# dazchi/gym-uav-collision-avoidance

Hardware: AMD Instinct MI355X
Metric: env-steps/s (higher is better)
Workload: dtype f32+f64

## Files before the change

gym_uav_collision_avoidance_amd/csrc/uavx_device.hpp:

```cpp
#pragma once
#include <hip/hip_runtime.h>
#include <stdint.h>

namespace uavx {

constexpr int kWave = 64;
#ifndef UAVX_BLOCK
#define UAVX_BLOCK 64
#endif
constexpr int kBlock = UAVX_BLOCK;
constexpr int kWavesPerBlock = kBlock / kWave;
constexpr float kPi = 3.14159265358979323846f;
constexpr float kInvPi = 0.318309886183790671538f;
constexpr float kTwoPi = 6.28318530717958647692f;
constexpr float kInvTwoPi = 0.159154943091895335769f;

__device__ __forceinline__ void wave_lds_sync() {
    __builtin_amdgcn_fence(__ATOMIC_RELEASE, "wavefront");
    __builtin_amdgcn_wave_barrier();
    __builtin_amdgcn_fence(__ATOMIC_ACQUIRE, "wavefront");
}

using rsrc_t = __amdgpu_buffer_rsrc_t;
typedef unsigned int u32x4 __attribute__((ext_vector_type(4)));
typedef unsigned int u32x2 __attribute__((ext_vector_type(2)));
constexpr int kAuxSc1 = 16;

__device__ __forceinline__ rsrc_t make_rsrc(const void *base, uint32_t bytes) {
    return __builtin_amdgcn_make_buffer_rsrc(const_cast<void *>(base),  0, (int)bytes, 0x00020000);
}
__device__ __forceinline__ void store16_wt(rsrc_t r, uint32_t byte_off, float4 v) {
    u32x4 d = {__float_as_uint(v.x), __float_as_uint(v.y), __float_as_uint(v.z), __float_as_uint(v.w)};
    __builtin_amdgcn_raw_buffer_store_b128(d, r, (int)byte_off, 0, kAuxSc1);
}
__device__ __forceinline__ void store16_wt(rsrc_t r, uint32_t byte_off, double2 v) {
    const unsigned long long a = __double_as_longlong(v.x), b = __double_as_longlong(v.y);
    u32x4 d = {(unsigned)a, (unsigned)(a >> 32), (unsigned)b, (unsigned)(b >> 32)};
    __builtin_amdgcn_raw_buffer_store_b128(d, r, (int)byte_off, 0, kAuxSc1);
}
__device__ __forceinline__ void store8_wt(rsrc_t r, uint32_t byte_off, float2 v) {
    u32x2 d = {__float_as_uint(v.x), __float_as_uint(v.y)};
    __builtin_amdgcn_raw_buffer_store_b64(d, r, (int)byte_off, 0, kAuxSc1);
}

typedef const __attribute__((address_space(4))) char *karg_ptr;
__device__ __forceinline__ karg_ptr late_kargs() {
    karg_ptr ka = (karg_ptr)__builtin_amdgcn_kernarg_segment_ptr();
    asm volatile("" : "+s"(ka));
    return ka;
}
template <class T>
__device__ __forceinline__ T late_karg(uint32_t byte_off, karg_ptr ka = late_kargs()) {
    return *(const __attribute__((address_space(4))) T *)(ka + byte_off);
}

__device__ __forceinline__ float sqrt_rn(float s) {
    if (__builtin_expect(__any((__float_as_uint(s) - 1u) < 0x0F7FFFFFu), 0)) return sqrtf(s);
    const float r = __builtin_amdgcn_sqrtf(s);
    const float lo = __uint_as_float(__float_as_uint(r) - 1u), hi = __uint_as_float(__float_as_uint(r) + 1u);
    const float e_lo = fmaf(-lo, r, s), e_hi = fmaf(-hi, r, s);
    float out = (e_lo <= 0.f) ? lo : r;
    out = (e_hi > 0.f) ? hi : out;
    return out;
}

__device__ __forceinline__ float norm32(float x, float y) {
    float a = x * x;
    float b = y * y;
    return sqrt_rn(a + b);
}

__device__ __forceinline__ double clip64(double x, double lo, double hi) {
    double m = (x < lo) ? lo : x;
    return (m > hi) ? hi : m;
}

__device__ __forceinline__ float wrap_pi(float x) {
    float k = rintf(x * kInvTwoPi);
    return fmaf(-k, kTwoPi, x);
}

__device__ __forceinline__ float atan2_fast(float y, float x) {
    const float ax = fabsf(x), ay = fabsf(y);
    const float mx = fmaxf(ax, ay), mn = fminf(ax, ay);
    const bool big = mn > 0.41421356237f * mx;
    const float num = big ? mn - mx : mn;
    float den = big ? mn + mx : mx;
    den = (mx == 0.f) ? 1.f : den;
    const float t = num * __builtin_amdgcn_rcpf(den);
    const float z = t * t;
    float pl = fmaf(8.05374449538e-2f, z, -1.38776856032e-1f);
    pl = fmaf(pl, z, 1.99777106478e-1f);
    pl = fmaf(pl, z, -3.33329491539e-1f);
    float r = fmaf(pl * z, t, t);
    r = big ? r + 0.78539816339744830962f : r;
    r = (ay > ax) ? 1.57079632679489661923f - r : r;
    r = (x < 0.f) ? kPi - r : r;
    return copysignf(r, y);
}

__device__ __forceinline__ float atan2_exact(float y, float x) {
    const float ax = fabsf(x), ay = fabsf(y);
    const float mx = fmaxf(ax, ay), mn = fminf(ax, ay);
    const bool big = mn > 0.41421356237f * mx;
    const float num = big ? mn - mx : mn;
    float den = big ? mn + mx : mx;
    den = (mx == 0.f) ? 1.f : den;
    const float t = num / den;
    const float z = t * t;
    float pl = fmaf(8.05374449538e-2f, z, -1.38776856032e-1f);
    pl = fmaf(pl, z, 1.99777106478e-1f);
    pl = fmaf(pl, z, -3.33329491539e-1f);
    float r = fmaf(pl * z, t, t);
    r = big ? r + 0.78539816339744830962f : r;
    r = (ay > ax) ? 1.57079632679489661923f - r : r;
    r = (x < 0.f) ? kPi - r : r;
    return copysignf(r, y);
}

__device__ __forceinline__ double max64u(double x, double lim) {
    double r;
    asm("v_max_f64 %0, %1, %2" : "=v"(r) : "v"(x), "s"(lim));
    return r;
}
__device__ __forceinline__ double min64u(double x, double lim) {
    double r;
    asm("v_min_f64 %0, %1, %2" : "=v"(r) : "v"(x), "s"(lim));
    return r;
}

__device__ __forceinline__ double div_tau(double x, double tau, double rtau, bool recip_ok) {
    if (!recip_ok) return x / tau;
    x = min64u(max64u(x, -1e300), 1e300);
    const double q0 = x * rtau;
    const double rem = fma(-q0, tau, x);
    return fma(rem, rtau, q0);
}

__device__ __forceinline__ void axis_update(double a, double tau, double rtau, bool recip_ok, double amax, double vmax,
                                            double &v, float &x) {
    const bool poisoned = __builtin_isunordered(a, v);
    const double dv = min64u(max64u(div_tau(a - v, tau, rtau, recip_ok), -amax), amax);
    double nv = min64u(max64u(v + dv * tau, -vmax), vmax);
    nv = poisoned ? __builtin_nan("") : nv;
    v = nv;
    x = (float)((double)x + v * tau);
}

__device__ __forceinline__ void sincospi32(float t, float &sn, float &cs) {
    const float k = rintf(2.0f * t);
    const float r = fmaf(-0.5f, k, t);
    const float z = r * r;
    float ps = fmaf(z, 0.0821458866f, -0.599264529f);
    ps = fmaf(ps, z, 2.55016404f);
    ps = fmaf(ps, z, -5.16771278f);
    ps = fmaf(ps, z, 3.14159265f);
    ps = ps * r;
    float pc = fmaf(z, -0.0258068913f, 0.235330630f);
    pc = fmaf(pc, z, -1.33526277f);
    pc = fmaf(pc, z, 4.05871213f);
    pc = fmaf(pc, z, -4.93480220f);
    pc = fmaf(pc, z, 1.0f);
    const int q = (int)k & 3;
    sn = (q == 0) ? ps : (q == 1) ? pc : (q == 2) ? -ps : -pc;
    cs = (q == 0) ? pc : (q == 1) ? -ps : (q == 2) ? -pc : ps;
}

__device__ __forceinline__ void sincos_ref(double x, double &sn, double &cs) {
    const double ax = fabs(x);
    if (__builtin_expect(__any(ax > 823549.6561538912), 0)) {
        if (ax > 823549.6561538912) { sincos(x, &sn, &cs); return; }
    }
    const double fn = rint(x * 6.36619772367581382433e-01);
    const int n = (int)fn;
    double r = x - fn * 1.57079632673412561417e+00;
    double t = r;
    double w = fn * 6.07710050630396597660e-11;
    r = t - w;
    w = fn * 2.02226624879595063154e-21 - ((t - r) - w);
    t = r;
    w = fn * 2.02226624871116645580e-21;
    r = t - w;
    w = fn * 8.47842766036889956997e-32 - ((t - r) - w);
    const double y0 = r - w;
    const double y1 = (r - y0) - w;
    const double z = y0 * y0, zz = z * z, v = z * y0;
    const double rs = 8.33333333332248946124e-03 + z * (-1.98412698298579493134e-04 + z * 2.75573137070700676789e-06) +
                      z * zz * (-2.50507602534068634195e-08 + z * 1.58969099521155010221e-10);
    const double ks = y0 - ((z * (0.5 * y1 - v * rs) - y1) - v * -1.66666666666666324348e-01);
    const double rc = z * (4.16666666666666019037e-02 + z * (-1.38888888888741095749e-03 + z * 2.48015872894767294178e-05)) +
                      zz * zz * (-2.75573143513906633035e-07 + z * (2.08757232129817482790e-09 + z * -1.13596475577881948265e-11));
    const double hz = 0.5 * z, wc = 1.0 - hz;
    const double kc = wc + (((1.0 - wc) - hz) + (z * rc - y0 * y1));
    const int q = n & 3;
    double s_ = (q == 0) ? ks : (q == 1) ? kc : (q == 2) ? -ks : -kc;
    double c_ = (q == 0) ? kc : (q == 1) ? -ks : (q == 2) ? -kc : ks;
    const bool tiny = ax < 7.450580596923828125e-9;
    s_ = tiny ? x : s_;
    c_ = tiny ? 1.0 : c_;
    const bool fin = ax <= 1.7976931348623157e308;
    sn = fin ? s_ : __builtin_nan("");
    cs = fin ? c_ : __builtin_nan("");
}

__device__ __forceinline__ void polar_to_command_ref32(float a0, float a1, float h, double &ax, double &ay) {
    const float u = a0 * 0.5f + 0.5f;
    const float v = u * h;
    const float theta = a1 * 3.14159265358979323846f;
    double s, c;
    sincos_ref((double)theta, s, c);
    ax = (double)(v * (float)c);
    ay = (double)(v * (float)s);
}
__device__ __forceinline__ void polar_to_command_ref64(double a0, double a1, float h, double &ax, double &ay) {
    const double v = (a0 * 0.5 + 0.5) * (double)h;
    const double theta = a1 * 3.14159265358979323846;
    double s, c;
    sincos_ref(theta, s, c);
    ax = v * c;
    ay = v * s;
}
template <bool ACT64>
__device__ __forceinline__ void polar_to_command_ref(float h, double &ax, double &ay) {
    if (ACT64) polar_to_command_ref64(ax, ay, h, ax, ay);
    else polar_to_command_ref32((float)ax, (float)ay, h, ax, ay);
}

__device__ __forceinline__ void philox4x32(uint32_t c0, uint32_t c1, uint32_t c2, uint32_t c3, uint32_t k0,
                                           uint32_t k1, uint32_t out[4]) {
#pragma unroll
    for (int r = 0; r < 10; r++) {
        uint64_t p0 = (uint64_t)0xD2511F53u * c0;
        uint64_t p1 = (uint64_t)0xCD9E8D57u * c2;
        uint32_t n0 = (uint32_t)(p1 >> 32) ^ c1 ^ k0;
        uint32_t n1 = (uint32_t)p1;
        uint32_t n2 = (uint32_t)(p0 >> 32) ^ c3 ^ k1;
        uint32_t n3 = (uint32_t)p0;
        c0 = n0; c1 = n1; c2 = n2; c3 = n3;
        k0 += 0x9E3779B9u; k1 += 0xBB67AE85u;
    }
    out[0] = c0; out[1] = c1; out[2] = c2; out[3] = c3;
}
__device__ __forceinline__ double bits53(uint32_t a, uint32_t b) {
    return ((double)(a >> 5) * 67108864.0 + (double)(b >> 6)) / 9007199254740992.0;
}
struct ResetCandidates {
    float sx, sy, tx, ty;
};
// ... 41 lines not shown
```

gym_uav_collision_avoidance_amd/csrc/uavx_multi.hip:

```cpp
#include <hip/hip_runtime.h>

#include <cmath>
#include <cstddef>
#include <cstdio>
#include <cstdlib>
#include <cstring>
#include <new>
#include <string>
#include <type_traits>

#include "../../include/uavx.h"
#include "uavx_device.hpp"

namespace uavx {

#ifndef UAVX_LATE
#define UAVX_LATE 1
#endif
template <bool ON>
__device__ __forceinline__ karg_ptr kargs_if() {
    if constexpr (ON && UAVX_LATE) return late_kargs();
    else return nullptr;
}
template <bool ON, class T>
// ... 147 lines not shown
    m.cnt = (int)envs_here * N;
    return m;
}
template <int NT, bool EXT = false, int W = 1>
__device__ __forceinline__ LaneMap lane_map(const MultiParams &p, uint32_t wave = blockIdx.x) {
    return lane_map_from<NT, EXT, W>((uint32_t)p.E, p.N, p.epw, p.magic, p.nslots, wave);
}

struct AgentRegs {
    float x, y, prev_d;
    uint32_t flags;
    float tx, ty, init_d;
    double vx, vy;
};

template <bool EXT, int W = 1>
struct LdsT {
    static constexpr int kW = W;
    static constexpr int kRows = (EXT && kExtSlots > kWave * W) ? kExtSlots : kWave * W;
    float4 pos[kRows];
    float theta[kRows];
    float obs[kWave * W * UAVX_OBS_DIM];
};
template <>
struct LdsT<true, 1> {
    static constexpr int kW = 1;
    static constexpr int kRows = kExtSlots;
    union {
        struct {
            float4 pos[kRows];
            float theta[kRows];
        };
        float obs[kWave * UAVX_OBS_DIM];
    };
};
template <int W>
__device__ __forceinline__ void group_sync() {
    if (W == 1) wave_lds_sync();
    else __syncthreads();
}
template <int W>
__device__ __forceinline__ bool group_any(bool v) {
    if (W == 1) return __ballot(v) != 0ull;
    return __syncthreads_or(v ? 1 : 0) != 0;
}
using Lds = LdsT<false>;
template <int T>
struct LdsTiles {
    static constexpr int kW = 1;
    static constexpr int kRows = kWave * T;
    float4 pos[kRows];
    float theta[kRows];
    float obs[kWave * T * UAVX_OBS_DIM];
};

template <bool EXT>
__device__ __forceinline__ float sense_limit(const MultiParams &p, uint32_t flags) {
    if (EXT && p.n_levels > 0) return p.levels[(flags & kLevelMask) >> kLevelShift].sq_sense;
    return p.sq_sense;
}
template <bool EXT>
__device__ __forceinline__ WorldLims world_lims(const MultiParams &p, uint32_t flags) {
    WorldLims w;
    if (EXT && p.n_levels > 0) {
        const float4 *t = reinterpret_cast<const float4 *>(&p.levels[(flags & kLevelMask) >> kLevelShift]);
        const float4 a = t[0], b = t[1];
        w.lo_x = a.x; w.lo_y = a.y; w.hi_x = a.z; w.hi_y = a.w;
        w.sq_sense = b.x; w.sq_two_r = b.y; w.inv_sense = b.z; w.inv_diag = b.w;
    } else {
        w.lo_x = p.lo_x; w.lo_y = p.lo_y; w.hi_x = p.hi_x; w.hi_y = p.hi_y;
        w.sq_sense = p.sq_sense; w.sq_two_r = p.sq_two_r; w.inv_sense = p.inv_sense; w.inv_diag = p.inv_diag;
    }
    return w;
}

__device__ __forceinline__ float natural_prev_d(uint32_t flags, float x, float y, float tx, float ty) {
    const float d = norm32(tx - x, ty - y);
    return ((flags & UAVX_FLAG_DONE) && !(flags & kFlagJustDone)) ? 0.f : d;
}

__device__ __forceinline__ void load_agent(const MultiParams &p, uint32_t a, AgentRegs &s) {
    const float2 d = p.pos[a];
    const double2 v = p.vel[a];
    const Goal g = p.goal[a];
    s.x = d.x; s.y = d.y;
    s.vx = v.x; s.vy = v.y;
    s.tx = g.tx; s.ty = g.ty; s.init_d = g.init_d; s.flags = g.flags;
    s.prev_d = natural_prev_d(s.flags, s.x, s.y, s.tx, s.ty);
    if (s.flags & kFlagPrevOvr) s.prev_d = p.prev_ovr[a];
}
__device__ __forceinline__ void store_agent(const MultiParams &p, float2 *pos, double2 *vel, Goal *goal, uint32_t a,
                                            const AgentRegs &s, uint32_t flags_in) {
    store16_wt(make_rsrc(vel, (uint32_t)p.E * (uint32_t)p.N * 16u), a * 16u, make_double2(s.vx, s.vy));
    pos[a] = make_float2(s.x, s.y);
    if (s.flags != flags_in) goal[a].flags = s.flags;
}
__device__ __forceinline__ void store_agent(const MultiParams &p, uint32_t a, const AgentRegs &s, uint32_t flags_in) {
    store_agent(p, p.pos, p.vel, p.goal, a, s, flags_in);
}

struct Neigh {
    float d1, d2;
    int j1, j2;
    float step_sq_min;
};

template <int NT, bool STEP, class LDS>
__device__ __forceinline__ Neigh scan_neighbours_exact(float sq_sense, const LaneMap &m, const LDS &lds, float nx,
                                                       float ny) {
    const int N = NT ? NT : m.nslots;
    Neigh r;
    r.d1 = r.d2 = INFINITY;
    r.j1 = r.j2 = -1;
    r.step_sq_min = INFINITY;
    const float4 *row = &lds.pos[m.rbase];
    auto visit = [&](int j, float4 q) {
        const float dxn = q.z - nx, dyn = q.w - ny;
        const float ax = dxn * dxn, ay = dyn * dyn;
        const float sn = ax + ay;
        if (STEP) {
            const float dxo = q.x - nx, dyo = q.y - ny;
            const float bx = dxo * dxo, by = dyo * dyo;
            const float so = bx + by;
            const float ss = (j < m.i) ? sn : so;
            r.step_sq_min = fminf(r.step_sq_min, (ss < sq_sense) ? ss : INFINITY);
        }
        const float dn = (sn < sq_sense) ? sqrt_rn(sn) : INFINITY;
        const bool lt1 = dn < r.d1, lt2 = dn < r.d2;
        r.d2 = lt1 ? r.d1 : (lt2 ? dn : r.d2);
        r.j2 = lt1 ? r.j1 : (lt2 ? j : r.j2);
        r.d1 = lt1 ? dn : r.d1;
        r.j1 = lt1 ? j : r.j1;
    };
    if (NT) {
        constexpr int M = NT > 1 ? NT - 1 : 1;
        float4 q[M];
        int js[M];
#pragma unroll
        for (int k = 0; k < NT - 1; k++) {
            js[k] = k + (k >= m.i ? 1 : 0);
            q[k] = row[js[k]];
        }
#pragma unroll
        for (int k = 0; k < NT - 1; k++) visit(js[k], q[k]);
    } else {
        for (int k = 0; k < N - 1; k++) {
            const int j = k + (k >= m.i ? 1 : 0);
            visit(j, row[j]);
        }
    }
    return r;
}

#ifdef UAVX_STAMPS
__shared__ int g_dbg_fallback;
#endif
__device__ __forceinline__ uint32_t med3_u32(uint32_t a, uint32_t b, uint32_t c) {
    uint32_t r;
    asm("v_med3_u32 %0, %1, %2, %3" : "=v"(r) : "v"(a), "v"(b), "v"(c));
    return r;
}

template <int NT, bool STEP, class LDS>
__device__ __forceinline__ Neigh scan_neighbours(float sq_sense, const LaneMap &m, const LDS &lds, float nx,
                                                 float ny) {
    if (NT != 0 && NT <= 5) return scan_neighbours_exact<NT, STEP>(sq_sense, m, lds, nx, ny);
    const int N = NT ? NT : m.nslots;
    if (NT == 0 && N <= 5) return scan_neighbours_exact<NT, STEP>(sq_sense, m, lds, nx, ny);
    const float4 *row = &lds.pos[m.rbase];
    uint32_t k1 = 0xffffffffu, k2 = 0xffffffffu, k3 = 0xffffffffu;
    float step_min = INFINITY;
    uint32_t keep;
    asm("v_mov_b32 %0, 0xffffffc0" : "=v"(keep));
    auto visit = [&](uint32_t c, bool below, float4 q) {
        const float dxn = q.z - nx, dyn = q.w - ny;
        const float ax = dxn * dxn, ay = dyn * dyn;
        const float sn = ax + ay;
        if (STEP) {
            const float dxo = q.x - nx, dyo = q.y - ny;
            const float bx = dxo * dxo, by = dyo * dyo;
            const float so = bx + by;
            step_min = fminf(step_min, below ? sn : so);
        }
        uint32_t key;
        asm("v_and_or_b32 %0, %1, %2, %3" : "=v"(key) : "v"(sn), "v"(keep), "s"(c));
        k3 = med3_u32(k2, k3, key);
        k2 = med3_u32(k1, k2, key);
        k1 = min(k1, key);
    };
    const char *rowb = reinterpret_cast<const char *>(row);
    auto other = [&](int c, bool below) {
        return *reinterpret_cast<const float4 *>(rowb + c * 16 + (below ? 0 : 16));
    };
    if (NT) {
#ifndef UAVX_SCANBATCH
#define UAVX_SCANBATCH 7
#endif
        constexpr int M = NT > 1 ? NT - 1 : 1;
        constexpr int BATCH = M < UAVX_SCANBATCH ? M : UAVX_SCANBATCH;
#pragma unroll
        for (int c0 = 0; c0 < NT - 1; c0 += BATCH) {
            float4 q[BATCH];
#pragma unroll
            for (int c = 0; c < BATCH; c++)
                if (c0 + c < NT - 1) q[c] = other(c0 + c, c0 + c < m.i);
#pragma unroll
            for (int c = 0; c < BATCH; c++)
                if (c0 + c < NT - 1) visit((uint32_t)(c0 + c), c0 + c < m.i, q[c]);
        }
    } else {
        const int NL = m.nlearn;
        int c = 0;
        for (; c + 1 < NL - 1; c += 2) {
            const bool la = c < m.i, lb = c + 1 < m.i;
            const float4 qa = other(c, la), qb = other(c + 1, lb);
            visit((uint32_t)c, la, qa);
            visit((uint32_t)c + 1u, lb, qb);
        }
        if (c < NL - 1) {
            const bool la = c < m.i;
            visit((uint32_t)c, la, other(c, la));
            c++;
        }
        auto body = [&](uint32_t c, int r) {
            const float2 q = *reinterpret_cast<const float2 *>(&row[r].z);
            const float dxn = q.x - nx, dyn = q.y - ny;
            const float ax = dxn * dxn, ay = dyn * dyn;
            const float sn = ax + ay;
            if (STEP) step_min = fminf(step_min, sn);
            uint32_t key;
            asm("v_and_or_b32 %0, %1, %2, %3" : "=v"(key) : "v"(sn), "v"(keep), "s"(c));
            k3 = med3_u32(k2, k3, key);
            k2 = med3_u32(k1, k2, key);
            k1 = min(k1, key);
        };
        for (; c + 1 < N - 1; c += 2) {
            body((uint32_t)c, c + 1);
            body((uint32_t)c + 1u, c + 2);
        }
        if (c < N - 1) body((uint32_t)c, c + 1);
    }
    const uint32_t t1 = k1 >> 6, t2 = k2 >> 6, t3 = k3 >> 6, ts = __float_as_uint(sq_sense) >> 6;
    const bool near_tie = m.active && ((t2 - t1 <= 1u && t1 <= ts) || (t3 - t2 <= 1u && t2 <= ts));
#ifdef UAVX_STAMPS
    if (__any(near_tie)) g_dbg_fallback = 1;
#endif
    const int c1 = (int)(k1 & 63u), c2 = (int)(k2 & 63u);
    const int j1 = c1 + (c1 >= m.i ? 1 : 0), j2 = c2 + (c2 >= m.i ? 1 : 0);
    const float4 q1 = row[j1], q2 = row[j2];
    const float ex1 = q1.z - nx, ey1 = q1.w - ny, ex2 = q2.z - nx, ey2 = q2.w - ny;
    const float mx1 = ex1 * ex1, my1 = ey1 * ey1, mx2 = ex2 * ex2, my2 = ey2 * ey2;
    const float s1 = mx1 + my1, s2 = mx2 + my2;
    const bool in1 = s1 < sq_sense, in2 = s2 < sq_sense;
    Neigh r;
    r.step_sq_min = (step_min < sq_sense) ? step_min : INFINITY;
    r.d1 = in1 ? sqrt_rn(s1) : INFINITY;
    r.d2 = in2 ? sqrt_rn(s2) : INFINITY;
    r.j1 = in1 ? j1 : -1;
    r.j2 = in2 ? j2 : -1;
    unsigned long long tied = __ballot(near_tie);
    if (__popcll(tied) > 6) return scan_neighbours_exact<NT, STEP>(sq_sense, m, lds, nx, ny);
    while (tied != 0ull) {
        const int tl = (int)__builtin_ctzll(tied);
        tied &= tied - 1ull;
        const float ax = __int_as_float(__builtin_amdgcn_readlane(__float_as_int(nx), tl));
        const float ay = __int_as_float(__builtin_amdgcn_readlane(__float_as_int(ny), tl));
        const float lim = __int_as_float(__builtin_amdgcn_readlane(__float_as_int(sq_sense), tl));
        const int ti = __builtin_amdgcn_readlane(m.i, tl), trb = __builtin_amdgcn_readlane(m.rbase, tl);
        const int t = (int)(threadIdx.x & (kWave - 1));
        const bool mine = t < N - 1;
        const int j = mine ? t + (t >= ti ? 1 : 0) : ti;
        const float4 q = lds.pos[trb + j];
        const float dx = q.z - ax, dy = q.w - ay;
        const float xx = dx * dx, yy = dy * dy;
        const float sn = xx + yy;
        const float dn = sqrt_rn(sn);
        unsigned long long key = (mine && sn < lim) ? ((unsigned long long)__float_as_uint(dn) << 32) | (uint32_t)j : ~0ull;
        auto wave_min = [](unsigned long long k) {
#pragma unroll
            for (int off = 32; off > 0; off >>= 1) {
                const uint32_t hi = __shfl_xor((uint32_t)(k >> 32), off), lo = __shfl_xor((uint32_t)k, off);
                const unsigned long long o = ((unsigned long long)hi << 32) | lo;
                k = o < k ? o : k;
            }
            return k;
        };
        const unsigned long long m1 = wave_min(key);
        const unsigned long long m2 = wave_min(key == m1 ? ~0ull : key);
        if (t == tl) {
            r.d1 = m1 == ~0ull ? INFINITY : __uint_as_float((uint32_t)(m1 >> 32));
            r.j1 = m1 == ~0ull ? -1 : (int)(uint32_t)m1;
            r.d2 = m2 == ~0ull ? INFINITY : __uint_as_float((uint32_t)(m2 >> 32));
            r.j2 = m2 == ~0ull ? -1 : (int)(uint32_t)m2;
        }
    }
    return r;
}

template <class LDS>
__device__ __forceinline__ void assemble_obs(const MultiParams &p, const WorldLims &w, const LaneMap &m, const LDS &lds,
                                             const Neigh &nb, float nx, float ny, float speed, float theta, float dist_t,
                                             float dth, float o[10]) {
    o[0] = speed * p.inv_vmax_norm;
    o[1] = theta * kInvPi;
    o[2] = dist_t * w.inv_diag;
    o[3] = dth * kInvPi;
    const bool has1 = nb.j1 >= 0, has2 = nb.j2 >= 0;
    const int i1 = m.rbase + (has1 ? nb.j1 : 0), i2 = m.rbase + (has2 ? nb.j2 : 0);
    const float4 q1 = lds.pos[i1], q2 = lds.pos[i2];
    const float t1 = lds.theta[i1], t2 = lds.theta[i2];
    const float b1 = wrap_pi(atan2_fast(q1.w - ny, q1.z - nx) - theta) * kInvPi;
    const float b2 = wrap_pi(atan2_fast(q2.w - ny, q2.z - nx) - theta) * kInvPi;
    const float h1 = wrap_pi(t1 - theta) * kInvPi;
    const float h2 = wrap_pi(t2 - theta) * kInvPi;
    o[4] = has1 ? nb.d1 * w.inv_sense : 1.f;
    o[5] = has1 ? b1 : 1.f;
    o[6] = has1 ? h1 : 0.f;
    o[7] = has2 ? nb.d2 * w.inv_sense : 1.f;
    o[8] = has2 ? b2 : 1.f;
    o[9] = has2 ? h2 : 0.f;
}

template <int NT, class LDS>
__device__ __forceinline__ void store_obs_block(const MultiParams &p, const LaneMap &m, LDS &lds, const float o[10],
                                                float *obs_out) {
    constexpr int T = kWave * LDS::kW;
    float *stage = lds.obs + m.obs0;
    if (m.active) {
        float2 *dst = reinterpret_cast<float2 *>(stage + m.lane * UAVX_OBS_DIM);
#pragma unroll
        for (int k = 0; k < 5; k++) dst[k] = make_float2(o[2 * k], o[2 * k + 1]);
    }
    group_sync<LDS::kW>();
    const int nfloat = m.cnt * UAVX_OBS_DIM;
    const rsrc_t r = make_rsrc(obs_out, (uint32_t)p.E * (uint32_t)p.N * (UAVX_OBS_DIM * 4u));
    const uint32_t gbase = m.a0 * (UAVX_OBS_DIM * 4u);
    if (NT ? (NT % 2 == 0) : ((p.N & 1) == 0)) {
#pragma unroll
        for (int k = 0; k < 3; k++) {
            const int f = (k * T + m.lane) * 4;
            if (f < nfloat) store16_wt(r, gbase + f * 4u, *reinterpret_cast<const float4 *>(stage + f));
        }
    } else {
        const int head = (gbase & 8u) ? 2 : 0;
        const int mid = (nfloat - head) / 4;
        const int tail = head + mid * 4;
#pragma unroll
        for (int k = 0; k < 3; k++) {
            const int q = k * T + m.lane;
            if (q < mid) {
                const float *src = stage + head + q * 4;
                const float2 lo = *reinterpret_cast<const float2 *>(src), hi = *reinterpret_cast<const float2 *>(src + 2);
                store16_wt(r, gbase + (uint32_t)(head + q * 4) * 4u, make_float4(lo.x, lo.y, hi.x, hi.y));
            }
        }
        if (m.lane == 0 && head) store8_wt(r, gbase, *reinterpret_cast<const float2 *>(stage));
        if (m.lane == 1 && tail < nfloat) store8_wt(r, gbase + (uint32_t)tail * 4u, *reinterpret_cast<const float2 *>(stage + tail));
    }
    group_sync<LDS::kW>();
}

__device__ __forceinline__ float4 make_leg(float body_step, float x, float y, float wx, float wy) {
    const float dx = wx - x, dy = wy - y;
    const float d = norm32(dx, dy);
    float4 leg = make_float4(0.f, 0.f, 0.f, 0.f);
    if (d > 0.f) {
        const float sc = body_step / d;
        leg.x = dx * sc; leg.y = dy * sc;
        leg.w = floorf(d / body_step);
    }
    leg.z = atan2_exact(dy, dx);
    return leg;
}

template <bool MOVE, class LDS, bool LATEW = false>
__device__ __forceinline__ void stage_bodies(const MultiParams &p, const LaneMap &m, LDS &lds, uint32_t flags, bool ready,
                                             uint32_t steps, uint32_t ep_draw) {
    const int L = p.N;
    const bool leveled = p.n_levels > 0;
    const LevelParams *lv = &p.levels[(flags & kLevelMask) >> kLevelShift];
    const int b_active = m.active ? (leveled ? lv->b_active : p.B) : 0;
    const uint32_t kk = steps & (uint32_t)p.body_pmask;
    const bool retarget = MOVE && steps != 0u && kk == 0u;
    const float kf = (float)kk;
#pragma unroll 1
    for (int k = 0; k < p.kb; k++) {
        const int b = k * L + m.i;
        const bool valid = m.active && b < p.B && !ready;
        const bool on = valid && b < b_active;
        const uint32_t gi = m.e * (uint32_t)p.B + (uint32_t)b;
        float2 q = make_float2(INFINITY, INFINITY);
        float4 leg = make_float4(0.f, 0.f, 0.f, 0.f);
        if (on) { q = p.body_pos[gi]; leg = p.body_leg[gi]; }
        if (on && retarget) {
            const ResetCandidates c = reset_candidates((uint64_t)LATE(LATEW, p, env_offset) + m.e, (uint32_t)(L + b),
                                                       0x80000000u | (steps >> p.body_pshift), ep_draw, LATE(LATEW, p, body_k0),
                                                       LATE(LATEW, p, body_k1), leveled ? lv->lox : LATE(LATEW, p, lox),
                                                       leveled ? lv->loy : LATE(LATEW, p, loy), leveled ? lv->hix : LATE(LATEW, p, hix),
                                                       leveled ? lv->hiy : LATE(LATEW, p, hiy));
            leg = make_leg(p.body_step, q.x, q.y, c.sx, c.sy);
            p.body_leg[gi] = leg;
        }
        if (MOVE && on && kf < leg.w) {
            q.x = q.x + leg.x; q.y = q.y + leg.y;
            p.body_pos[gi] = q;
        }
        if (valid) {
            lds.pos[m.rbase + L + b] = make_float4(q.x, q.y, q.x, q.y);
            lds.theta[m.rbase + L + b] = leg.z;
        }
    }
}

template <int NT, bool EXT, class LDS, bool LATEW = false>
__device__ __forceinline__ void step_agent(const MultiParams &p, const LaneMap &m, LDS &lds, AgentRegs &s, double ax,
                                           double ay, int evaluate, float o[10], float &rew, uint32_t &done_out,
                                           uint32_t &reach_ev, uint32_t &coll_ev, bool frozen = false,
                                           uint32_t env_steps = 0, uint32_t ep_draw = 0) {
    const float sq_sense = sense_limit<EXT>(p, s.flags);
    const bool was_done = (s.flags & UAVX_FLAG_DONE) != 0;
    const bool parked = EXT && (s.flags & kFlagInactive) != 0;
    if (!frozen) s.flags &= ~(kFlagPrevOvr | kFlagJustDone);
    const float ox = s.x, oy = s.y;
    float pd = 0.f, d = 0.f;
    if (!was_done && !frozen && !parked) {
        axis_update(ax, p.tau, p.rtau, p.recip_ok != 0, p.amax, p.vmax, s.vx, s.x);
        axis_update(ay, p.tau, p.rtau, p.recip_ok != 0, p.amax, p.vmax, s.vy, s.y);
        pd = s.prev_d;
    }
    const float tdx = s.tx - s.x, tdy = s.ty - s.y;
    const float dist_t = norm32(tdx, tdy);
    if (!was_done) d = dist_t;
    const float theta = atan2_fast((float)s.vy, (float)s.vx);
    const float dth = wrap_pi(atan2_fast(tdy, tdx) - theta);

    if (m.active) {
        lds.pos[m.rbase + m.i] = make_float4(ox, oy, s.x, s.y);
        lds.theta[m.rbase + m.i] = theta;
    }
    if (EXT && p.B > 0) stage_bodies<true, LDS, LATEW>(p, m, lds, s.flags, frozen, env_steps, ep_draw);
    group_sync<LDS::kW>();
    const Neigh nb = scan_neighbours<NT, true>(sq_sense, m, lds, s.x, s.y);
    const WorldLims w = world_lims<EXT>(p, s.flags);

    const float inv_init = __builtin_amdgcn_rcpf(s.init_d);
    float r = -0.01f * fminf(p.vmax_norm * inv_init, 1.0f);
    r += (50.0f * p.inv_vmax_norm) * (pd - d);
    const float frac = d * inv_init * (1.0f / 1.5f);
    r *= (r > 0.f) ? (1.0f - frac) : (1.0f + frac);
    r -= 0.01f * fabsf(dth);

    const bool collision = nb.step_sq_min <= w.sq_two_r;
    if (collision) r = -2.0f;
    coll_ev = 0;
    if (nb.step_sq_min <= p.sq_hard && !(s.flags & (UAVX_FLAG_DONE | UAVX_FLAG_COLLIDED)) && !frozen) {
        coll_ev = 1;
        s.flags |= UAVX_FLAG_COLLIDED;
    }
    const double sq = fma(s.vy, s.vy, s.vx * s.vx);
    const bool oob = !(s.x >= w.lo_x && s.x <= w.hi_x && s.y >= w.lo_y && s.y <= w.hi_y);
    float speed = __builtin_amdgcn_sqrtf((float)sq);
    reach_ev = 0;
    if (frozen) {
        done_out = 0;
        r = 0.f;
    } else if (d < 0.5f && !collision && sq < p.speed_sq_lim) {
        done_out = 1;
        reach_ev = was_done ? 0u : 1u;
        s.flags |= UAVX_FLAG_DONE | (was_done ? 0u : kFlagJustDone);
        const double nv = sqrt(sq);
        double fx = s.vx / nv * 0.001, fy = s.vy / nv * 0.001;
        if (fx != fx || fy != fy) { fx = 0.0; fy = 0.0; }
        s.vx = fx; s.vy = fy;
        speed = __builtin_amdgcn_sqrtf((float)fma(fy, fy, fx * fx));
        r += 10.0f;
    } else if (oob) {
        done_out = evaluate ? 0u : 1u;
    } else {
        done_out = 0;
    }
    if (!frozen) s.prev_d = d;
    rew = r;
    assemble_obs(p, w, m, lds, nb, s.x, s.y, speed, theta, dist_t, dth, o);
    if (parked) {
#pragma unroll
        for (int k = 0; k < UAVX_OBS_DIM; k++) o[k] = 0.f;
        rew = 0.f;
        done_out = frozen ? 0u : 1u;
    }
}

template <bool ACT64>
__device__ __forceinline__ void load_action(const void *__restrict__ actions, uint32_t a, double &ax, double &ay) {
    if (ACT64) {
        const double2 v = reinterpret_cast<const double2 *>(actions)[a];
        ax = v.x; ay = v.y;
    } else {
        const float2 v = reinterpret_cast<const float2 *>(actions)[a];
        ax = (double)v.x; ay = (double)v.y;
    }
}

#ifndef UAVX_STEPB
#define UAVX_STEPB 8
#endif
template <int NT, bool ACT64, bool EXT, int W, int T = 1>
__global__ __launch_bounds__(kWave * W * T, (EXT && W == 1) ? UAVX_STEPB : 1) void step_kernel(
    const void *__restrict__ actions, char *slab, uint32_t off_vel, uint32_t off_goal, uint32_t off_rec, uint32_t off_wsteps,
    uint32_t num_envs, uint32_t n_agents, uint32_t envs_per_group, uint32_t magic, uint32_t nslots, MultiParams p, int evaluate,
    float *__restrict__ obs_out, float *__restrict__ rew_out, uint8_t *__restrict__ done_out) {
    static_assert(T == 1 || W == 1, "tiles are one-wavefront workgroups side by side");
    using LDS = std::conditional_t<(T > 1), LdsTiles<T>, LdsT<EXT, W>>;
    static_assert(T == 1 || !EXT, "tiles: the plain variants only");
    __shared__ LDS lds;
    const uint32_t tile = T > 1 ? (uint32_t)__builtin_amdgcn_readfirstlane((int)(threadIdx.x / kWave)) : 0u;
    float2 *const pos_b = reinterpret_cast<float2 *>(slab);
    double2 *const vel_b = reinterpret_cast<double2 *>(slab + off_vel);
    Goal *const goal_b = reinterpret_cast<Goal *>(slab + off_goal);
    const uint32_t wave_id = blockIdx.x * T + tile;
    const LaneMap m = lane_map_from<NT, EXT, W>(num_envs, (int)n_agents, (int)envs_per_group, (int)magic, (int)nslots, wave_id,
                                                T > 1 ? threadIdx.x % kWave : threadIdx.x, tile);
    AgentRegs s = {};
    double ax = 0.0, ay = 0.0;
    uint4 rec = make_uint4(0, 0, 0, 0);
    uint32_t wave_count = 0;
    {
        const uint32_t el = m.active ? m.e : 0u, al = m.active ? m.a : 0u;
        if (EXT) {
            rec = reinterpret_cast<const uint4 *>(slab + off_rec)[el];
            wave_count = reinterpret_cast<const uint32_t *>(slab + off_wsteps)[wave_id];
        }
        load_action<ACT64>(actions, al, ax, ay);
        const float2 d = pos_b[al];
        const double2 v = vel_b[al];
        const Goal g = goal_b[al];
        __builtin_amdgcn_sched_barrier(0);
        s.x = d.x; s.y = d.y; s.vx = v.x; s.vy = v.y;
        s.tx = g.tx; s.ty = g.ty; s.init_d = g.init_d; s.flags = g.flags;
        s.prev_d = natural_prev_d(s.flags, s.x, s.y, s.tx, s.ty);
        if (m.active && (s.flags & kFlagPrevOvr)) s.prev_d = p.prev_ovr[m.a];
    }
    const uint32_t flags_in = s.flags;
    float o[10], rew;
    uint32_t dn, re, ce;
    step_agent<NT, EXT, LDS, false>(p, m, lds, s, ax, ay, evaluate, o, rew, dn, re, ce, false, wave_count - rec.x,
                                    ((rec.y & ~kRecEnded) - 1u) & ~kRecEnded);
    if (m.active) {
        if (!(EXT && (flags_in & kFlagInactive))) store_agent(p, pos_b, vel_b, goal_b, m.a, s, flags_in);
        rew_out[m.a] = rew;
        done_out[m.a] = (uint8_t)dn;
        if (re) atomicAdd(&p.reach[m.e], 1u);
        if (ce) atomicAdd(&p.coll[m.e], 1u);
        if (!(fabsf(rew) < INFINITY)) atomicAdd(&p.nonfin[m.e], 1u);
        if (m.lane == 0) {
            uint32_t *const ws = reinterpret_cast<uint32_t *>(slab + off_wsteps);
            if (EXT) ws[m.wave] = wave_count + 1u;
            else atomicAdd(&ws[m.wave], 1u);
        }
    }
    store_obs_block<NT>(p, m, lds, o, obs_out);
}

template <class LDS, class MAP>
__device__ __forceinline__ bool lowest_clash(const MAP &m, LDS &lds, unsigned long long group, bool clash, int &low) {
    if (LDS::kW == 1) {
        const unsigned long long bits = __ballot(clash);
        const unsigned long long mine = (bits >> m.base) & group;
        low = mine ? (int)__builtin_ctzll(mine) : 64;
        return bits != 0ull;
    } else {
        int *slot = reinterpret_cast<int *>(lds.obs) + m.g;
        if (m.i == 0) *slot = 64;
        __syncthreads();
        if (clash) atomicMin(slot, m.i);
        const bool any = __syncthreads_or(clash ? 1 : 0) != 0;
        low = *slot;
        return any;
    }
}

__device__ __forceinline__ bool too_close(float sq_two_r, float ax, float ay, float bx, float by) {
    const float dx = ax - bx, dy = ay - by;
    const float xx = dx * dx, yy = dy * dy;
    return xx + yy <= sq_two_r;
}

#ifndef UAVX_CHAINROWS
#define UAVX_CHAINROWS 4
#endif
constexpr int kChainRows = UAVX_CHAINROWS;
template <int NT, bool EXT, class LDS>
__device__ __forceinline__ void reset_envs_wave(const MultiParams &p, const LaneMap &m, LDS &lds, bool go,
                                                uint32_t episode, uint32_t k0, uint32_t k1, AgentRegs &s,
                                                float2 *bpos_out, float4 *bleg_out, uint8_t *lvl_out) {
    const int N = NT ? NT : p.N;
    float4 *row = &lds.pos[m.rbase];
    const uint64_t ge = (uint64_t)p.env_offset + m.e;
    const unsigned long long group = (N >= 64) ? ~0ull : ((1ull << N) - 1ull);
    double lox = p.lox, loy = p.loy, hix = p.hix, hiy = p.hiy;
    float sq2r = p.sq_two_r;
    uint32_t lvl = 0;
    int nl = N, nb = 0;
    if (EXT) {
        if (go && p.n_levels > 0) {
            if (p.level_lo >= 0) {
                uint32_t o[4];
                reset_words(ge, 0xFFFFu, 0u, episode, k0, k1, o);
                lvl = (uint32_t)p.level_lo + __umulhi(o[0], (uint32_t)(p.level_hi - p.level_lo + 1));
            } else {
                lvl = p.lvl_next[m.e];
            }
            lvl = min(lvl, (uint32_t)(p.n_levels - 1));
        }
        nb = p.B;
        if (p.n_levels > 0) {
            const LevelParams *lv = &p.levels[lvl];
            lox = lv->lox; loy = lv->loy; hix = lv->hix; hiy = lv->hiy;
            sq2r = lv->sq_two_r;
            nl = lv->n_active; nb = lv->b_active;
        }
    }
    const bool gl = go && m.i < nl;
    ResetCandidates c = {0.f, 0.f, 0.f, 0.f};
    if (gl) {
        c = reset_candidates(ge, m.i, 0u, episode, k0, k1, lox, loy, hix, hiy);
        row[m.i] = make_float4(c.sx, c.sy, c.tx, c.ty);
    }
    group_sync<LDS::kW>();
#pragma unroll 1
    for (int phase = 0; phase < 2; phase++) {
        uint32_t attempt = 0;
#pragma unroll 1
        for (;;) {
            bool clash = false;
            if (gl) {
                const float qx = phase ? c.tx : c.sx, qy = phase ? c.ty : c.sy;
                clash = phase ? too_close(sq2r, qx, qy, c.sx, c.sy) : false;
#pragma unroll 1
                for (int j0 = 0; j0 < m.i; j0 += kChainRows) {
                    float2 o[kChainRows];
#pragma unroll
                    for (int u = 0; u < kChainRows; u++) {
                        const float4 *r4 = &row[min(j0 + u, m.i - 1)];
                        o[u] = *reinterpret_cast<const float2 *>(phase ? &r4->z : &r4->x);
                    }
#pragma unroll
                    for (int u = 0; u < kChainRows; u++) clash = clash || too_close(sq2r, o[u].x, o[u].y, qx, qy);
                }
            }
            int low;
            if (!lowest_clash<LDS>(m, lds, group, clash, low)) break;
            const bool redraw = gl && m.i == low;
            group_sync<LDS::kW>();
            if (redraw) {
                const ResetCandidates r = reset_candidates(ge, m.i, ++attempt, episode, k0, k1, lox, loy, hix, hiy);
                if (phase) { c.tx = r.tx; c.ty = r.ty; row[m.i].z = c.tx; row[m.i].w = c.ty; }
                else { c.sx = r.sx; c.sy = r.sy; row[m.i].x = c.sx; row[m.i].y = c.sy; }
            }
            group_sync<LDS::kW>();
        }
    }
    if (EXT) {
#pragma unroll 1
        for (int k = 0; k < p.kb; k++) {
            const int b = k * N + m.i;
            const bool on = go && b < nb;
            const int slot = N + b;
            uint32_t attempt = 0;
            float qx = 0.f, qy = 0.f;
            if (on) {
                const ResetCandidates r = reset_candidates(ge, (uint32_t)slot, 0u, episode, k0, k1, lox, loy, hix, hiy);
                qx = r.sx; qy = r.sy;
                row[slot].x = qx; row[slot].y = qy;
            }
            group_sync<LDS::kW>();
#pragma unroll 1
            for (;;) {
                bool clash = false;
                if (on) {
                    const int cnt = nl + b;
#pragma unroll 1
                    for (int j0 = 0; j0 < cnt; j0 += kChainRows) {
                        float2 o[kChainRows];
#pragma unroll
                        for (int u = 0; u < kChainRows; u++) {
                            const int j = min(j0 + u, cnt - 1);
                            o[u] = *reinterpret_cast<const float2 *>(&row[j < nl ? j : N + (j - nl)].x);
                        }
#pragma unroll
                        for (int u = 0; u < kChainRows; u++) clash = clash || too_close(sq2r, o[u].x, o[u].y, qx, qy);
                    }
                }
                int low;
                if (!lowest_clash<LDS>(m, lds, group, clash, low)) break;
                const bool redraw = on && m.i == low;
                group_sync<LDS::kW>();
                if (redraw) {
                    const ResetCandidates r = reset_candidates(ge, (uint32_t)slot, ++attempt, episode, k0, k1, lox, loy, hix, hiy);
                    qx = r.sx; qy = r.sy;
                    row[slot].x = qx; row[slot].y = qy;
                }
                group_sync<LDS::kW>();
            }
// ... 1562 lines not shown
```

Baseline: 10.82 billion.

## Add squared-distance neighbour scan, buffer loads, cheaper atan2 and angle wrap

```diff
diff --git a/gym_uav_collision_avoidance_amd/csrc/uavx_device.hpp b/gym_uav_collision_avoidance_amd/csrc/uavx_device.hpp
--- a/gym_uav_collision_avoidance_amd/csrc/uavx_device.hpp
+++ b/gym_uav_collision_avoidance_amd/csrc/uavx_device.hpp
@@ -80,20 +80,21 @@
     return fmaf(-k, kTwoPi, x);
 }
 
+__device__ __forceinline__ float wrap_unit(float x) {
+    return fmaf(__builtin_amdgcn_fractf(fmaf(x, kInvTwoPi, 0.5f)), 2.0f, -1.0f);
+}
+
 __device__ __forceinline__ float atan2_fast(float y, float x) {
     const float ax = fabsf(x), ay = fabsf(y);
     const float mx = fmaxf(ax, ay), mn = fminf(ax, ay);
-    const bool big = mn > 0.41421356237f * mx;
-    const float num = big ? mn - mx : mn;
-    float den = big ? mn + mx : mx;
-    den = (mx == 0.f) ? 1.f : den;
-    const float t = num * __builtin_amdgcn_rcpf(den);
+    const float t = mn * __builtin_amdgcn_rcpf(fmaxf(mx, 1.17549435e-38f));
     const float z = t * t;
-    float pl = fmaf(8.05374449538e-2f, z, -1.38776856032e-1f);
-    pl = fmaf(pl, z, 1.99777106478e-1f);
-    pl = fmaf(pl, z, -3.33329491539e-1f);
+    float pl = fmaf(7.37447338e-3f, z, -3.55211943e-2f);
+    pl = fmaf(pl, z, 8.21691155e-2f);
+    pl = fmaf(pl, z, -1.33988619e-1f);
+    pl = fmaf(pl, z, 1.98618680e-1f);
+    pl = fmaf(pl, z, -3.33253950e-1f);
     float r = fmaf(pl * z, t, t);
-    r = big ? r + 0.78539816339744830962f : r;
     r = (ay > ax) ? 1.57079632679489661923f - r : r;
     r = (x < 0.f) ? kPi - r : r;
     return copysignf(r, y);
diff --git a/gym_uav_collision_avoidance_amd/csrc/uavx_multi.hip b/gym_uav_collision_avoidance_amd/csrc/uavx_multi.hip
--- a/gym_uav_collision_avoidance_amd/csrc/uavx_multi.hip
+++ b/gym_uav_collision_avoidance_amd/csrc/uavx_multi.hip
@@ -323,9 +323,6 @@
     return r;
 }
 
-#ifdef UAVX_STAMPS
-__shared__ int g_dbg_fallback;
-#endif
 __device__ __forceinline__ uint32_t med3_u32(uint32_t a, uint32_t b, uint32_t c) {
     uint32_t r;
     asm("v_med3_u32 %0, %1, %2, %3" : "=v"(r) : "v"(a), "v"(b), "v"(c));
@@ -333,8 +330,61 @@
 }
 
 template <int NT, bool STEP, class LDS>
+__device__ __forceinline__ Neigh scan_neighbours_sq(float sq_sense, const LaneMap &m, const LDS &lds, float nx, float ny) {
+    static_assert(NT == 4, "three other agents");
+    const float4 *row = &lds.pos[m.rbase];
+    constexpr uint32_t kInfBits = 0x7f800000u;
+    uint32_t s1 = kInfBits, s2 = kInfBits, s3 = kInfBits;
+    float step_min = INFINITY;
+    int j1 = -1, j2 = -1;
+    constexpr int M = NT - 1;
+    float4 q[M];
+    int js[M];
+#pragma unroll
+    for (int k = 0; k < M; k++) {
+        js[k] = k + (k >= m.i ? 1 : 0);
+        q[k] = row[js[k]];
+    }
+#pragma unroll
+    for (int k = 0; k < M; k++) {
+        const int j = js[k];
+        const float dxn = q[k].z - nx, dyn = q[k].w - ny;
+        const float ax = dxn * dxn, ay = dyn * dyn;
+        const float sn0 = ax + ay;
+        if (STEP) {
+            const float dxo = q[k].x - nx, dyo = q[k].y - ny;
+            const float bx = dxo * dxo, by = dyo * dyo;
+            const float so = bx + by;
+            step_min = fminf(step_min, (j < m.i) ? sn0 : so);
+        }
+        const uint32_t sn = (sn0 < sq_sense) ? __float_as_uint(sn0) : kInfBits;
+        const bool lt1 = sn < s1, lt2 = sn < s2;
+        j2 = lt1 ? j1 : (lt2 ? j : j2);
+        j1 = lt1 ? j : j1;
+        s3 = med3_u32(s2, s3, sn);
+        s2 = med3_u32(s1, s2, sn);
+        s1 = min(s1, sn);
+    }
+    Neigh r;
+    r.step_sq_min = (step_min < sq_sense) ? step_min : INFINITY;
+    r.d1 = sqrt_rn(__uint_as_float(s1));
+    r.d2 = sqrt_rn(__uint_as_float(s2));
+    const bool swap = r.d1 == r.d2 && j2 < j1;
+    r.j1 = swap ? j2 : j1;
+    r.j2 = swap ? j1 : j2;
+    const bool near_tie = m.active && s3 < kInfBits && s3 - s2 <= 8u;
+    if (__builtin_expect(__any(near_tie), 0)) return scan_neighbours_exact<NT, STEP>(sq_sense, m, lds, nx, ny);
+    return r;
+}
+
+#ifdef UAVX_STAMPS
+__shared__ int g_dbg_fallback;
+#endif
+
+template <int NT, bool STEP, class LDS, bool SQ = false>
 __device__ __forceinline__ Neigh scan_neighbours(float sq_sense, const LaneMap &m, const LDS &lds, float nx,
                                                  float ny) {
+    if (SQ && NT == 4) return scan_neighbours_sq<4, STEP>(sq_sense, m, lds, nx, ny);
     if (NT != 0 && NT <= 5) return scan_neighbours_exact<NT, STEP>(sq_sense, m, lds, nx, ny);
     const int N = NT ? NT : m.nslots;
     if (NT == 0 && N <= 5) return scan_neighbours_exact<NT, STEP>(sq_sense, m, lds, nx, ny);
@@ -480,10 +530,10 @@
     const int i1 = m.rbase + (has1 ? nb.j1 : 0), i2 = m.rbase + (has2 ? nb.j2 : 0);
     const float4 q1 = lds.pos[i1], q2 = lds.pos[i2];
     const float t1 = lds.theta[i1], t2 = lds.theta[i2];
-    const float b1 = wrap_pi(atan2_fast(q1.w - ny, q1.z - nx) - theta) * kInvPi;
-    const float b2 = wrap_pi(atan2_fast(q2.w - ny, q2.z - nx) - theta) * kInvPi;
-    const float h1 = wrap_pi(t1 - theta) * kInvPi;
-    const float h2 = wrap_pi(t2 - theta) * kInvPi;
+    const float b1 = wrap_unit(atan2_fast(q1.w - ny, q1.z - nx) - theta);
+    const float b2 = wrap_unit(atan2_fast(q2.w - ny, q2.z - nx) - theta);
+    const float h1 = wrap_unit(t1 - theta);
+    const float h2 = wrap_unit(t2 - theta);
     o[4] = has1 ? nb.d1 * w.inv_sense : 1.f;
     o[5] = has1 ? b1 : 1.f;
     o[6] = has1 ? h1 : 0.f;
@@ -583,7 +633,7 @@
     }
 }
 
-template <int NT, bool EXT, class LDS, bool LATEW = false>
+template <int NT, bool EXT, class LDS, bool LATEW = false, bool SQ = false>
 __device__ __forceinline__ void step_agent(const MultiParams &p, const LaneMap &m, LDS &lds, AgentRegs &s, double ax,
                                            double ay, int evaluate, float o[10], float &rew, uint32_t &done_out,
                                            uint32_t &reach_ev, uint32_t &coll_ev, bool frozen = false,
@@ -611,7 +661,7 @@
     }
     if (EXT && p.B > 0) stage_bodies<true, LDS, LATEW>(p, m, lds, s.flags, frozen, env_steps, ep_draw);
     group_sync<LDS::kW>();
-    const Neigh nb = scan_neighbours<NT, true>(sq_sense, m, lds, s.x, s.y);
+    const Neigh nb = scan_neighbours<NT, true, LDS, SQ>(sq_sense, m, lds, s.x, s.y);
     const WorldLims w = world_lims<EXT>(p, s.flags);
 
     const float inv_init = __builtin_amdgcn_rcpf(s.init_d);
@@ -685,9 +735,14 @@
     static_assert(T == 1 || !EXT, "tiles: the plain variants only");
     __shared__ LDS lds;
     const uint32_t tile = T > 1 ? (uint32_t)__builtin_amdgcn_readfirstlane((int)(threadIdx.x / kWave)) : 0u;
+    constexpr bool BUF = NT == 4 && !EXT && T == 1;
     float2 *const pos_b = reinterpret_cast<float2 *>(slab);
     double2 *const vel_b = reinterpret_cast<double2 *>(slab + off_vel);
     Goal *const goal_b = reinterpret_cast<Goal *>(slab + off_goal);
+    const uint32_t nslot = num_envs * n_agents;
+    const rsrc_t r_act = make_rsrc(actions, nslot * (ACT64 ? 16u : 8u));
+    const rsrc_t r_pos = make_rsrc(slab, nslot * 8u), r_vel = make_rsrc(slab + off_vel, nslot * 16u);
+    const rsrc_t r_goal = make_rsrc(slab + off_goal, nslot * 16u);
     const uint32_t wave_id = blockIdx.x * T + tile;
     const LaneMap m = lane_map_from<NT, EXT, W>(num_envs, (int)n_agents, (int)envs_per_group, (int)magic, (int)nslots, wave_id,
                                                 T > 1 ? threadIdx.x % kWave : threadIdx.x, tile);
@@ -701,25 +756,51 @@
             rec = reinterpret_cast<const uint4 *>(slab + off_rec)[el];
             wave_count = reinterpret_cast<const uint32_t *>(slab + off_wsteps)[wave_id];
         }
-        load_action<ACT64>(actions, al, ax, ay);
-        const float2 d = pos_b[al];
-        const double2 v = vel_b[al];
-        const Goal g = goal_b[al];
-        __builtin_amdgcn_sched_barrier(0);
-        s.x = d.x; s.y = d.y; s.vx = v.x; s.vy = v.y;
-        s.tx = g.tx; s.ty = g.ty; s.init_d = g.init_d; s.flags = g.flags;
+        if (!BUF) {
+            load_action<ACT64>(actions, al, ax, ay);
+            const float2 d = pos_b[al];
+            const double2 v = vel_b[al];
+            const Goal g = goal_b[al];
+            __builtin_amdgcn_sched_barrier(0);
+            s.x = d.x; s.y = d.y; s.vx = v.x; s.vy = v.y;
+            s.tx = g.tx; s.ty = g.ty; s.init_d = g.init_d; s.flags = g.flags;
+        } else {
+            if (ACT64) {
+                const u32x4 c = __builtin_amdgcn_raw_buffer_load_b128(r_act, al * 16u, 0, 0);
+                ax = __hiloint2double(c.y, c.x); ay = __hiloint2double(c.w, c.z);
+            } else {
+                const u32x2 c = __builtin_amdgcn_raw_buffer_load_b64(r_act, al * 8u, 0, 0);
+                ax = (double)__uint_as_float(c.x); ay = (double)__uint_as_float(c.y);
+            }
+            const u32x2 d = __builtin_amdgcn_raw_buffer_load_b64(r_pos, al * 8u, 0, 0);
+            const u32x4 v = __builtin_amdgcn_raw_buffer_load_b128(r_vel, al * 16u, 0, 0);
+            const u32x4 g = __builtin_amdgcn_raw_buffer_load_b128(r_goal, al * 16u, 0, 0);
+            __builtin_amdgcn_sched_barrier(0);
+            s.x = __uint_as_float(d.x); s.y = __uint_as_float(d.y);
+            s.vx = __hiloint2double(v.y, v.x); s.vy = __hiloint2double(v.w, v.z);
+            s.tx = __uint_as_float(g.x); s.ty = __uint_as_float(g.y); s.init_d = __uint_as_float(g.z); s.flags = g.w;
+        }
         s.prev_d = natural_prev_d(s.flags, s.x, s.y, s.tx, s.ty);
         if (m.active && (s.flags & kFlagPrevOvr)) s.prev_d = p.prev_ovr[m.a];
     }
     const uint32_t flags_in = s.flags;
     float o[10], rew;
     uint32_t dn, re, ce;
-    step_agent<NT, EXT, LDS, false>(p, m, lds, s, ax, ay, evaluate, o, rew, dn, re, ce, false, wave_count - rec.x,
+    step_agent<NT, EXT, LDS, false, BUF>(p, m, lds, s, ax, ay, evaluate, o, rew, dn, re, ce, false, wave_count - rec.x,
                                     ((rec.y & ~kRecEnded) - 1u) & ~kRecEnded);
     if (m.active) {
-        if (!(EXT && (flags_in & kFlagInactive))) store_agent(p, pos_b, vel_b, goal_b, m.a, s, flags_in);
-        rew_out[m.a] = rew;
-        done_out[m.a] = (uint8_t)dn;
+        if (!BUF) {
+            if (!(EXT && (flags_in & kFlagInactive))) store_agent(p, pos_b, vel_b, goal_b, m.a, s, flags_in);
+            rew_out[m.a] = rew;
+            done_out[m.a] = (uint8_t)dn;
+        } else {
+            store16_wt(r_vel, m.a * 16u, make_double2(s.vx, s.vy));
+            const u32x2 d = {__float_as_uint(s.x), __float_as_uint(s.y)};
+            __builtin_amdgcn_raw_buffer_store_b64(d, r_pos, m.a * 8u, 0, 0);
+            if (s.flags != flags_in) __builtin_amdgcn_raw_buffer_store_b32(s.flags, r_goal, m.a * 16u + 12u, 0, 0);
+            __builtin_amdgcn_raw_buffer_store_b32(__float_as_uint(rew), make_rsrc(rew_out, nslot * 4u), m.a * 4u, 0, 0);
+            __builtin_amdgcn_raw_buffer_store_b8((uint8_t)dn, make_rsrc(done_out, nslot), m.a, 0, 0);
+        }
         if (re) atomicAdd(&p.reach[m.e], 1u);
         if (ce) atomicAdd(&p.coll[m.e], 1u);
         if (!(fabsf(rew) < INFINITY)) atomicAdd(&p.nonfin[m.e], 1u);
```

New measurement: 11.17 billion (median of 6 runs). 1.03x the previous value.
